# cselab/odil

Measured on AMD Instinct MI355X. Metric: grid-point-updates/s, Poisson 512^3 multigrid, higher is better.
Workload: dtype f64; 1 GPU; 3D Poisson 512^3 multigrid (9 levels) Adam epoch, 1xMI355X, public operator API (odil.util.optimize_grad on examples/poisson/poisson.py); cells_per_gpu=134217728, levels=9, optimizer=adam lr=0.005, decomposition=none, rccl_ranks=1, exchanges_per_epoch=0

## Files before the change

include/odil_hip.h:

```cpp
#ifndef ODIL_HIP_H
#define ODIL_HIP_H

#include <stddef.h>
#include <stdint.h>

#ifdef __cplusplus
extern "C" {
#endif

#define ODIL_MAX_NDIM 4
#define ODIL_MAX_LEVELS 32
#define ODIL_E_INVAL (-1)
#define ODIL_E_LAUNCH (-2)
#define ODIL_E_NODEV (-3)

const char* odil_last_error(void);
int odil_version(void);
int odil_device_count(void);
size_t odil_reduce_workspace_bytes(void);

int odil_interp_add_f64(const double* coarse, const double* add, double* fine, const int64_t* cshape, int ndim,
                        const char* loc, double coarse_scale, double add_scale, void* stream);
int odil_interp_add_f32(const float* coarse, const float* add, float* fine, const int64_t* cshape, int ndim,
                        const char* loc, float coarse_scale, float add_scale, void* stream);
// ... 84 lines not shown
int odil_poisson_residual_restrict_slab_f64(const double* u, const double* rhs, double* coarse, const int64_t* shape,
                                            int ndim, const double* h2, double scale, int64_t z0, int64_t z1,
                                            double denom, double* partials, double* loss, void* stream);
int odil_poisson_residual_restrict_slab_f32(const float* u, const float* rhs, float* coarse, const int64_t* shape,
                                            int ndim, const float* h2, float scale, int64_t z0, int64_t z1, double denom,
                                            double* partials, float* loss, void* stream);
int odil_poisson_adjoint_transpose_adam_f64(const double* fu, double* g0, double* g1, const int64_t* fshape,
                                            const double* h2, double scale, double* x0, double* m0, double* v0,
                                            double* x1, double* m1, double* v1, double alpha, double one_minus_b1,
                                            double one_minus_b2, double eps, const double* alpha_dev, int cut_lo,
                                            int cut_hi, void* stream);
int odil_poisson_adjoint_transpose_adam_f32(const float* fu, float* g0, float* g1, const int64_t* fshape,
                                            const float* h2, float scale, float* x0, float* m0, float* v0, float* x1,
                                            float* m1, float* v1, float alpha, float one_minus_b1, float one_minus_b2,
                                            float eps, const float* alpha_dev, int cut_lo, int cut_hi, void* stream);
int odil_poisson_jacobi_f64(const double* u, const double* rhs, double* uout, const int64_t* shape, int ndim,
                            const double* h2, double omega, void* stream);
int odil_poisson_jacobi_f32(const float* u, const float* rhs, float* uout, const int64_t* shape, int ndim,
                            const float* h2, float omega, void* stream);

int odil_poisson_jacobi2_f64(const double* u, const double* rhs, double* uout, const int64_t* shape, int ndim,
                             const double* h2, double omega1, double omega2, int zc_hint, void* stream);
int odil_poisson_jacobi2_f32(const float* u, const float* rhs, float* uout, const int64_t* shape, int ndim,
                             const float* h2, float omega1, float omega2, int zc_hint, void* stream);

int odil_poisson_jacobi2_synth_f64(const double* coarse, const double* x, const double* rhs, double* xout,
                                   const int64_t* cshape, const double* h2, double omega1, double omega2, int zc_hint,
                                   void* stream);
int odil_poisson_jacobi2_synth_f32(const float* coarse, const float* x, const float* rhs, float* xout,
                                   const int64_t* cshape, const float* h2, float omega1, float omega2, int zc_hint,
// ... 267 lines not shown
```

odil_amd/_lib.py:

```python

import ctypes
import os
from ctypes import c_char_p, c_double, c_float, c_int, c_int64, c_size_t, c_void_p

import numpy as np
import torch

_HERE = os.path.dirname(os.path.abspath(__file__))
LIB_PATH = os.environ.get("ODIL_HIP_LIB") or os.path.join(_HERE, "libodil_hip.so")

_P = c_void_p
_I64P = ctypes.POINTER(c_int64)

_R = "real"
_SIGNATURES = {
    "interp_add": [_P, _P, _P, _I64P, c_int, c_char_p, _R, _R, _P],
    "interp_adj": [_P, _P, _P, _I64P, c_int, c_char_p, _R, _P],
    "interp_add_ld": [_P, c_int64, _P, _P, _I64P, c_int, c_char_p, _R, _R, _P],
    "interp_adj_ld": [_P, _P, c_int64, _I64P, c_int, c_char_p, _P],
    "interp_adj_cut": [_P, _P, _P, _I64P, c_int, c_char_p, _R, c_int, c_int, _P],
    "interp_adj_cut_adam": [_P, _P, _I64P, c_int, c_char_p, c_int, c_int, _P, _P, _P, _R, _R, _R, _R, _P, _P],
    "restrict": [_P, _P, _I64P, c_int, c_char_p, _P],
    "restrict_adj": [_P, _P, _I64P, c_int, c_char_p, _P],
    "conv_valid": [_P, _P, _P, _I64P, _I64P, _I64P, _I64P, c_int, c_int, _P],
# ... 16 lines not shown
    "poisson_adjoint_adam_volumes": [_P, _P, _P, _P, _P, c_int, c_int64, c_int64, c_int64, c_int64, c_int64, _I64P, c_int,
                                     _P, _R, _R, _R, _R, _P, c_int64, _P],
    "mg_synth_adj_adam_volumes": [_P, _P, _I64P, c_int, c_int, c_int, _P, _P, _P, _R, _R, _R, _P, c_int64, _P],
    "poisson_jacobi": [_P, _P, _P, _I64P, c_int, _P, _R, _P],
    "poisson_jacobi2": [_P, _P, _P, _I64P, c_int, _P, _R, _R, c_int, _P],
    "poisson_jacobi2_synth": [_P, _P, _P, _P, _I64P, _P, _R, _R, c_int, _P],
    "poisson_residual_restrict": [_P, _P, _P, _I64P, c_int, _P, _R, _P, _P, _P],
    "poisson_residual_restrict_slab": [_P, _P, _P, _I64P, c_int, _P, _R, c_int64, c_int64, c_double, _P, _P, _P],
    "poisson_residual_synth": [_P, _P, _P, _P, _I64P, _P, c_int64, c_int64, c_double, _P, _P, c_size_t, _P, _P],
    "poisson_jacobi_synth": [_P, _P, _P, _P, _I64P, _P, _R, _P],
    "poisson_residual_slab": [_P, _P, _P, _I64P, c_int, _P, c_int64, c_int64, c_double, _P, _P, _P],
    "poisson_adjoint": [_P, _P, _I64P, c_int, _P, _R, _P],
    "poisson_adjoint_adam": [_P, _P, _P, _P, _P, _I64P, c_int, _P, _R, _R, _R, _R, _R, _P, _P],
    "poisson_adjoint_transpose_adam": [_P, _P, _P, _I64P, _P, _R, _P, _P, _P, _P, _P, _P, _R, _R, _R, _R, _P, c_int,
                                       c_int, _P],
    "poisson_jac_coeffs": [_P, _I64P, c_int, _P, _P],
    "poisson_jac_match": [_P, _I64P, c_int, _P, _P, _P, _P],
    "adam_step": [_P, _P, _P, _P, c_int64, _R, _R, _R, _R, _P, _P],
    "adam_step_pieces": [_P, _P, _P, _P, c_int64, c_int64, c_int64, c_int64, _R, _R, _R, _R, _P, _P],
    "planes_copy": [_P, _P, _P, c_int, c_int64, c_int, c_int, _P],
    "axpy": [_P, _P, c_int64, _R, _P],
    "scale": [_P, _P, c_int64, _R, _P, _P],
    "addcmul": [_P, _P, _P, c_int64, c_int, _P],
    "dots": [_P, c_int64, c_int, _P, c_int64, _P, _P, _P],
    "dots3": [_P, c_int64, c_int, _P, _P, _P, c_int64, _P, _P, _P],
    "lbfgs_probe": [_P, _P, c_int64, _P, _P, _P],
    "lincomb": [_P, _R, _P, c_int64, c_int, _P, c_int64, _P],
    "stencil_apply": [_P, _I64P, c_int, _P, _P, _I64P, c_int, c_int, _P],
    "stencil_march": [_P, _I64P, c_int, c_int, _P, _P, _I64P, c_int, c_int, c_int, _P],
    "stencil_var_smooth": [_P, _P, _P, _P, _I64P, c_int, _R, c_int, _P],
# ... 16 lines not shown
    "bmg_transfer": [_I64P, _I64P, _P, _P, _P, _P, c_int, _P],
    "bmg_galerkin": [_I64P, _I64P, _P, _P, _P, _P, c_int, c_int64, _P, _P],
}

_SIGNATURES_F64 = {
    "bmg_coarse_dense": [_P, _P, _I64P, c_int64, c_int64, _P, _P],
    "bmg_coarse_chol": [_P, c_int64, c_int64, c_double, _P, _P, _P, _P],
}

EXPORTED = [
    "odil_last_error", "odil_version", "odil_device_count", "odil_reduce_workspace_bytes", "odil_dots_workspace_bytes",
    "odil_dense_block_workspace_bytes", "odil_dense_block_wide_workspace_bytes", "odil_narrow_scale", "odil_widen_axpy",
    "odil_poisson_small_epochs_resident", "odil_poisson_small_epochs_partials", "odil_poisson_batch_partials",
    "odil_mg_batch_levels_ok", "odil_poisson_residual_synth_workspace_bytes",
    "odil_mg_volumes_levels_ok", "odil_interp_adj_kind", "odil_poisson_residual_synth_batch_workspace_bytes",
    "odil_poisson_residual_synth_batch_partials", "odil_stencil_solve_batch_work",
] + [
    "odil_{}_{}".format(name, suffix) for name in _SIGNATURES for suffix in ("f64", "f32")
] + ["odil_{}_f64".format(name) for name in _SIGNATURES_F64]

_lib = None


class OdilHipError(RuntimeError):
    pass


def load():
    global _lib
    if _lib is not None:
        return _lib
# ... 21 lines not shown
    lib.odil_poisson_batch_partials.argtypes = [_I64P, c_int, c_int]
    lib.odil_mg_batch_levels_ok.restype = c_int
    lib.odil_mg_batch_levels_ok.argtypes = [_I64P, c_int, c_int, c_int]
    lib.odil_poisson_residual_synth_workspace_bytes.restype = c_size_t
    lib.odil_poisson_residual_synth_workspace_bytes.argtypes = [_I64P]
    lib.odil_interp_adj_kind.restype = c_int
    lib.odil_interp_adj_kind.argtypes = [_I64P, c_int, c_char_p, c_int]
    lib.odil_mg_volumes_levels_ok.restype = c_int
    lib.odil_mg_volumes_levels_ok.argtypes = [_I64P, c_int, c_int, c_int, c_int]
    lib.odil_poisson_residual_synth_batch_workspace_bytes.restype = c_size_t
    lib.odil_poisson_residual_synth_batch_workspace_bytes.argtypes = [_I64P]
    lib.odil_poisson_residual_synth_batch_partials.restype = c_int64
    lib.odil_poisson_residual_synth_batch_partials.argtypes = [_I64P]
    lib.odil_stencil_solve_batch_work.restype = c_int64
    lib.odil_stencil_solve_batch_work.argtypes = [_I64P, c_int, c_int]
    for name in ("odil_narrow_scale", "odil_widen_axpy"):
        fn = getattr(lib, name)
        fn.restype = c_int
        fn.argtypes = [_P, _P, c_int64, c_double, _P, _P]
    for name, sig in _SIGNATURES.items():
        for suffix, real in (("f64", c_double), ("f32", c_float)):
            fn = getattr(lib, "odil_{}_{}".format(name, suffix))
            fn.restype = c_int
            fn.argtypes = [real if a is _R else a for a in sig]
    for name, sig in _SIGNATURES_F64.items():
        fn = getattr(lib, "odil_{}_f64".format(name))
        fn.restype = c_int
        fn.argtypes = sig
    _lib = lib
    return lib
# ... 71 lines not shown
```

odil_amd/csrc/common.h:

```cpp
#pragma once

#include <hip/hip_runtime.h>
#include <stdint.h>
#include <stdio.h>
#include <string.h>

#include "odil_hip.h"

namespace odil {

constexpr int kNumXcd = 8;
constexpr int kBlock = 256;
constexpr int kMaxPartials = 65536;
constexpr int kDotPartials = 1024;
constexpr int64_t kStreamBytes = (int64_t)128 << 20;
constexpr int kGridCap = 2048;

void set_error(const char* fmt, ...);

inline int check_launch(const char* what) {
  hipError_t err = hipGetLastError();
  if (err != hipSuccess) {
    set_error("%s: %s", what, hipGetErrorString(err));
    return ODIL_E_LAUNCH;
// ... 58 lines not shown
  int64_t per_xcd = (int64_t)s.Z * s.Yc * s.XS;
  int64_t cap = kGridCap / kNumXcd;
  if (per_xcd > cap) per_xcd = cap;
  if (per_xcd < 1) per_xcd = 1;
  return (int)(per_xcd * kNumXcd);
}

struct UnitSched {
  int ZCH, Y, XS;
  int ZC;
  int axis;
  int chunk;
  int per_xcd;
};

inline UnitSched make_unit_sched_chunked(int64_t Z, int64_t Y, int64_t XS, int zc) {
  UnitSched s;
  s.ZC = zc;
  s.ZCH = (int)((Z + zc - 1) / zc);
  s.Y = (int)Y;
  s.XS = (int)XS;
  if (Y >= 4 * kNumXcd) {
    s.axis = 1;
    s.chunk = (int)((Y + kNumXcd - 1) / kNumXcd);
    s.per_xcd = s.ZCH * s.chunk * s.XS;
  } else if (s.ZCH >= kNumXcd) {
    s.axis = 0;
    s.chunk = 0;
    s.per_xcd = (int)(((int64_t)s.ZCH * s.Y * s.XS + kNumXcd - 1) / kNumXcd);
  } else {
    s.axis = -1;
    s.chunk = 0;
    s.per_xcd = s.ZCH * s.Y * s.XS;
  }
  return s;
}

inline UnitSched make_unit_sched(int64_t Z, int64_t Y, int64_t XS, int64_t target_units = 2 * kGridCap) {
  int64_t zc = (Z * Y * XS) / target_units;
  if (zc < 1) zc = 1;
  if (zc > 64) zc = 64;
  if (zc > Z) zc = Z;
  return make_unit_sched_chunked(Z, Y, XS, (int)zc);
}

inline int unit_grid(const UnitSched& s) { return s.axis < 0 ? s.per_xcd : s.per_xcd * kNumXcd; }

#ifdef __HIPCC__
__device__ inline bool unit_decode(const UnitSched& s, int& zc, int& y, int& xs) {
  if (s.axis < 0) {
    const int i = blockIdx.x;
    xs = i % s.XS;
    const int r = i / s.XS;
    y = r % s.Y;
    zc = r / s.Y;
    return true;
  }
  const int k = blockIdx.x % kNumXcd, i = blockIdx.x / kNumXcd;
  xs = i % s.XS;
  const int r = i / s.XS;
  if (s.axis == 1) {
    y = k * s.chunk + r % s.chunk;
    zc = r / s.chunk;
    return y < s.Y;
  }
  const int u = k * s.per_xcd + i;
  xs = u % s.XS;
  const int ru = u / s.XS;
  y = ru % s.Y;
  zc = ru / s.Y;
  return zc < s.ZCH;
}
#endif

#ifdef __HIPCC__
struct RowIter {
  int t, step, count, y0, ny;
};

__device__ inline RowIter sched_begin(const RowSched& s) {
  RowIter it;
  const int k = blockIdx.x % kNumXcd;
  it.t = blockIdx.x / kNumXcd;
  it.step = gridDim.x / kNumXcd;
  it.y0 = k * s.Yc;
  int y1 = it.y0 + s.Yc;
  if (y1 > s.Y) y1 = s.Y;
  it.ny = y1 > it.y0 ? y1 - it.y0 : 0;
// ... 78 lines not shown
```

odil_amd/csrc/mg_march.hip:

```cpp
#include "mg_march.h"
#include "poisson.h"

namespace odil {

template <typename T, int CX>
__device__ inline void acc_plane(T (&s)[2][2 * CX], const T (&v)[3][CX + 2], int wz) {
#pragma unroll
  for (int sy = 0; sy < 2; ++sy)
#pragma unroll
    for (int sx = 0; sx < 2 * CX; ++sx) {
      T t = s[sy][sx];
#pragma unroll
      for (int ry = 0; ry < 2; ++ry)
#pragma unroll
        for (int rx = 0; rx < 2; ++rx) {
          const int w = wz * (sy == ry ? 1 : 3) * ((sx & 1) == rx ? 1 : 3);
          t = t + T(w) * v[sy + ry][(sx >> 1) + (sx & 1) + rx];
        }
      s[sy][sx] = t;
    }
}

template <typename T, int CX>
__device__ inline void zero_plane(T (&s)[2][2 * CX]) {
// ... 846 lines not shown
                                           typename TileVec<T, CX>::type (&pre)[2][kTileLoads], T (&wc)[CX][6],
                                           T (&wr)[CX][6], const AdamArgs<T>& ad, const float* __restrict__ wt) {
  __syncthreads();
#pragma unroll
  for (int i = 0; i < kTileLoads; ++i) {
    tile0[dst[i]] = pre[0][i];
    tile1[dst[i]] = pre[1][i];
  }
  __syncthreads();
  tile_fetch<T, CX>(c.gfine, 2 * (c.z0 - 1 + k + ahead), c.fnz, c.fplane, src, pre);
  tile_reduce_emit<T, CX>(c, tile0, tile1, k, live, wc, wr, ad, wt);
}

template <typename T, int CX>
__global__ __launch_bounds__(kBlock) void k_interp_adj_tile(const T* __restrict__ gfine, T* __restrict__ gcoarse,
                                                            T* __restrict__ gscaled, MarchArgs a, T scale,
                                                            AdamArgs<T> ad) {
  typedef typename TileVec<T, CX>::type P2;
  constexpr int NV = 2 * CX;
  __shared__ P2 tile[2][kTileLds];
  __shared__ float wtab[12 * (CX + 1) * kBlock];
  const int cny = a.cn[1], fny = a.fn[1], fnx = a.fn[2];
  int zc, yt, xt;
  if (!unit_decode(a.usched, zc, yt, xt)) return;
  TileCtx<T> c;
  c.cnz = a.cn[0], c.cnx = a.cn[2], c.fnz = a.fn[0];
  c.cut_lo = a.cut_lo, c.cut_hi = a.cut_hi;
  c.cplane = (int64_t)cny * c.cnx, c.fplane = (int64_t)fny * fnx;
  const int64_t cvol = (int64_t)blockIdx.y * c.cnz * c.cplane, fvol = (int64_t)blockIdx.y * c.fnz * c.fplane;
  gfine += fvol;
  c.gfine = gfine, c.gcoarse = gcoarse + cvol, c.gscaled = gscaled ? gscaled + cvol : nullptr;
  if (ad.x) ad.x += cvol, ad.m += cvol, ad.v += cvol;
  if (ad.alpha_dev) ad.alpha_dev += (int64_t)blockIdx.y * ad.alpha_stride;
  c.scale = scale;
  c.z0 = zc * a.usched.ZC;
  const int z1 = c.z0 + a.usched.ZC < c.cnz ? c.z0 + a.usched.ZC : c.cnz;
  tile_column(c.lx, c.ly);
  c.jy = yt * kTileY + c.ly, c.jx = (xt * kTileX + c.lx) * CX;
  c.owner = c.jy < cny && c.jx < c.cnx;
  c.cny = cny;
  c.sx = c.owner && (c.jx < 2 || c.jx + CX - 1 >= c.cnx - 2);
  c.sy = c.owner && (c.jy < 2 || c.jy >= cny - 2);
  if (c.sx || c.sy) {
    Adj6 ax[CX];
    column_taps<CX>(c.jx, c.cnx, ax);
    tile_tables_store<CX>(wtab, adj6(c.jy, cny), ax);
  }
  int64_t src[kTileLoads];
  int dst[kTileLoads];
#pragma unroll
  for (int k = 0; k < kTileLoads; ++k) {
// ... 50 lines not shown
      const int p = threadIdx.x + i * kBlock;
      if (p < kFuPacks) slot[p] = scale * pre[q][i];
    }
  }
}

template <typename T, bool MUL>
__device__ __forceinline__ T lap_inner(T fb, T fm, T fp, const H2<T>& h, int ax) {
  const T s = (fp + fm) + T(-2) * fb;
  if constexpr (MUL) return s * h.inv[ax];
  return div_h2<T>(s, h, ax);
}

template <typename T, bool MUL, bool G0>
__global__ __launch_bounds__(kBlock) void k_poisson_adjoint_tile(const T* __restrict__ fu, T* __restrict__ g0out_,
                                                                 T* __restrict__ gcoarse, MarchArgs a, H2<T> h,
                                                                 T scale, AdamArgs<T> ad0, T* __restrict__ x1,
                                                                 T* __restrict__ m1, T* __restrict__ v1) {
  T* const g0out = G0 ? g0out_ : nullptr;
  AdamArgs<T> ad1 = ad0;
  ad1.x = x1, ad1.m = m1, ad1.v = v1;
  typedef typename TileVec<T>::type P2;
  __shared__ P2 ring[4 * kFuPacks];
  __shared__ P2 gt[2][kTileR * kTileRS];
  const int cny = a.cn[1], fny = a.fn[1], fnx = a.fn[2];
  int zc, yt, xt;
  if (!unit_decode(a.usched, zc, yt, xt)) return;
  if constexpr (MUL) h.mul_ok[0] = h.mul_ok[1] = h.mul_ok[2] = 1;
  if (ad0.alpha_dev) ad0.alpha = *ad0.alpha_dev;
  ad0.alpha_dev = nullptr;
  ad1.alpha = ad0.alpha, ad1.alpha_dev = nullptr;
  TileCtx<T> c;
  c.gfine = nullptr, c.gcoarse = gcoarse, c.gscaled = nullptr;
  c.cnz = a.cn[0], c.cnx = a.cn[2], c.fnz = a.fn[0];
  c.cut_lo = a.cut_lo, c.cut_hi = a.cut_hi;
  c.cplane = (int64_t)cny * c.cnx, c.fplane = (int64_t)fny * fnx;
  c.scale = T(1);
  c.z0 = zc * a.usched.ZC;
  const int z1 = c.z0 + a.usched.ZC < c.cnz ? c.z0 + a.usched.ZC : c.cnz;
  tile_column(c.lx, c.ly);
  c.jy = yt * kTileY + c.ly, c.jx = xt * kTileX + c.lx;
  c.owner = c.jy < cny && c.jx < c.cnx;
  c.cny = cny;
  c.sx = c.owner && (c.jx < 2 || c.jx >= c.cnx - 2);
  c.sy = c.owner && (c.jy < 2 || c.jy >= cny - 2);
  const int fy0 = 2 * yt * kTileY, fx0 = 2 * xt * kTileX;
  const bool tile_inner = fy0 >= 4 && fy0 + 2 * kTileY + 4 <= fny && fx0 >= 4 && fx0 + 2 * kTileX + 4 <= fnx;
  int64_t src[kFuLoads];
#pragma unroll
  for (int i = 0; i < kFuLoads; ++i) {
    int p = threadIdx.x + i * kBlock;
    p = p < kFuPacks ? p : kFuPacks - 1;
    const int r = p / kFuC, cc = p - r * kFuC;
    int fy = fy0 - 3 + r, fx = fx0 - 4 + 2 * cc;
// ... 542 lines not shown
template <typename T>
static bool adj_rows_launch(const T* gfine, T* gcoarse, T* gscaled, const MarchArgs& m, T scale, hipStream_t stream,
                            const AdamArgs<T>& ad) {
  if constexpr (sizeof(T) != 4) {
    return false;
  } else {
    RowsArgs r;
    if (!adj_rows_plan<T>(m, aligned_to(gfine, 16), aligned_to(gcoarse, 8), r)) return false;
    hipLaunchKernelGGL(k_interp_adj_rows, dim3((unsigned)(r.per_xcd * kNumXcd)), dim3(kBlock), 0, stream, gfine, gcoarse,
                       gscaled, r, scale, ad);
    return true;
  }
}

template <typename T>
static void launch_adj_tile(dim3 grid, bool wide, hipStream_t stream, const T* gfine, T* gcoarse, T* gscaled,
                            const MarchArgs& m, T scale, const AdamArgs<T>& ad) {
  if constexpr (sizeof(T) == 4) {
    if (wide) {
      hipLaunchKernelGGL((k_interp_adj_tile<T, 2>), grid, dim3(kBlock), 0, stream, gfine, gcoarse, gscaled, m, scale, ad);
      return;
    }
  }
  hipLaunchKernelGGL((k_interp_adj_tile<T, 1>), grid, dim3(kBlock), 0, stream, gfine, gcoarse, gscaled, m, scale, ad);
}

static bool adj_tile_enabled() {
  const char* e = getenv("ODIL_ADJ_TILE");
  return !e || atoi(e) != 0;
}

static bool adj_small_level(const InterpArgs& a) { return a.cn[0] * a.cn[1] * a.cn[2] * a.cn[3] <= ((int64_t)1 << 22); }

static bool adj_tile_serves(const MarchArgs& m, const InterpArgs& a, int cx) {
  return cx == 1 && m.cn[1] >= 2 * kTileY && m.cn[2] >= 2 * kTileX && adj_tile_enabled() && !a.coarse_ld;
}

template <typename T>
int interp_adj_kind(const InterpArgs& a) {
// ... 17 lines not shown
  const dim3 grid(unit_grid(m.usched), m.lead_cn);
  const bool tile_ok = adj_tile_serves(m, a, CX);
  const bool tile_wide = sizeof(T) == 4 && m.cn[2] % 2 == 0 && m.cn[2] >= 4 * kTileX && aligned_to(gfine, 16);
  const int tile_cols = kTileX * (tile_wide ? 2 : 1);
  if (m.lead_fn != 1) {
    if (m.lead_loc == kNode)
      hipLaunchKernelGGL((k_interp_adj_march_lead<T, CX, 3>), grid, dim3(kBlock), 0, stream, gfine, gcoarse, gscaled,
                         m, scale, ad);
    else if (adj_rows_launch<T>(gfine, gcoarse, gscaled, m, scale, stream, ad)) {
    } else if (tile_ok) {
      const int64_t ytiles = (m.cn[1] + kTileY - 1) / kTileY, xtiles = (m.cn[2] + tile_cols - 1) / tile_cols;
      m.tx = kTileX;
      m.ty = kTileY;
      const int64_t per_volume = kGridCap / m.lead_cn > 2 * ytiles * xtiles ? kGridCap / m.lead_cn : 2 * ytiles * xtiles;
      m.usched = make_unit_sched(m.cn[0], ytiles, xtiles, per_volume);
      launch_adj_tile<T>(dim3(unit_grid(m.usched), m.lead_cn), tile_wide, stream, gfine, gcoarse, gscaled, m, scale, ad);
    } else
      hipLaunchKernelGGL((k_interp_adj_march_lead<T, CX, 1>), grid, dim3(kBlock), 0, stream, gfine, gcoarse, gscaled,
                         m, scale, ad);
  } else if (a.loc[1] == kNode)
    hipLaunchKernelGGL((k_interp_adj_march_n<T, CX>), grid, dim3(kBlock), 0, stream, gfine, gcoarse, gscaled, m, scale,
                       ad);
  else if (adj_rows_launch<T>(gfine, gcoarse, gscaled, m, scale, stream, ad)) {
  } else if (tile_ok) {
    const int64_t ytiles = (m.cn[1] + kTileY - 1) / kTileY, xtiles = (m.cn[2] + tile_cols - 1) / tile_cols;
    m.tx = kTileX;
    m.ty = kTileY;
    m.usched = make_unit_sched(m.cn[0], ytiles, xtiles, small_level ? ODIL_ADJ_UNITS_SMALL : ODIL_TILE_UNITS);
    launch_adj_tile<T>(dim3(unit_grid(m.usched)), tile_wide, stream, gfine, gcoarse, gscaled, m, scale, ad);
  } else
    hipLaunchKernelGGL((k_interp_adj_march<T, CX>), grid, dim3(kBlock), 0, stream, gfine, gcoarse, gscaled, m, scale,
                       ad);
  const int e = check_launch("k_interp_adj_march");
  return e ? e : 1;
}

template <typename T>
int poisson_adjoint_transpose(const T* fu, T* g0, T* g1, const int64_t* fshape, const T* h2, T scale,
                              const AdamArgs<T>& ad0, const AdamArgs<T>& ad1, int cut_lo, int cut_hi,
                              hipStream_t stream) {
  if (!fu || !g1 || !fshape || !h2) {
    set_error("poisson_adjoint_transpose: null pointer (fu, g1, shape, h2)");
    return ODIL_E_INVAL;
  }
  MarchArgs m;
  for (int i = 0; i < 3; ++i) {
    if (fshape[i] < 4 || fshape[i] % 2 || fshape[i] >= (1 << 30)) {
      set_error("poisson_adjoint_transpose: extent %lld on axis %d must be even, >= 4", (long long)fshape[i], i);
      return ODIL_E_INVAL;
    }
    m.fn[i] = (int)fshape[i];
    m.cn[i] = (int)(fshape[i] / 2);
  }
  const void* ptrs[] = {fu, g0, g1, ad0.x, ad0.m, ad0.v};
  for (const void* q : ptrs)
    if (q && !aligned_to(q, 2 * sizeof(T))) {
      set_error("poisson_adjoint_transpose: arrays must be aligned to %d bytes", (int)(2 * sizeof(T)));
      return ODIL_E_INVAL;
    }
  m.tx = kTileX, m.ty = kTileY;
  m.cut_lo = cut_lo, m.cut_hi = cut_hi;
  m.nt = 0;
  m.lead_loc = 0, m.lead_cn = 1, m.lead_fn = 1;
  const int64_t ytiles = (m.cn[1] + kTileY - 1) / kTileY, xtiles = (m.cn[2] + kTileX - 1) / kTileX;
  if ((int64_t)m.cn[0] * ytiles * xtiles >= ((int64_t)1 << 31)) {
    set_error("poisson_adjoint_transpose: grid too large for one launch");
    return ODIL_E_INVAL;
  }
  m.usched = make_unit_sched(m.cn[0], ytiles, xtiles, 2 * kGridCap);
  T h[3] = {h2[0], h2[1], h2[2]};
  const H2<T> hh = make_h2<T>(h);
  const bool mul = hh.mul_ok[0] && hh.mul_ok[1] && hh.mul_ok[2];
  const dim3 grid(unit_grid(m.usched));
#define ODIL_LAUNCH_ADJ_TILE(MUL, G0)                                                                             \
  hipLaunchKernelGGL((k_poisson_adjoint_tile<T, MUL, G0>), grid, dim3(kBlock), 0, stream, fu, g0, g1, m, hh, scale, \
                     ad0, ad1.x, ad1.m, ad1.v)
  if (mul && !g0) ODIL_LAUNCH_ADJ_TILE(true, false);
  else if (mul) ODIL_LAUNCH_ADJ_TILE(true, true);
  else if (!g0) ODIL_LAUNCH_ADJ_TILE(false, false);
  else ODIL_LAUNCH_ADJ_TILE(false, true);
#undef ODIL_LAUNCH_ADJ_TILE
  return check_launch("k_poisson_adjoint_tile");
}

template int poisson_adjoint_transpose<double>(const double*, double*, double*, const int64_t*, const double*, double,
                                               const AdamArgs<double>&, const AdamArgs<double>&, int, int, hipStream_t);
template int poisson_adjoint_transpose<float>(const float*, float*, float*, const int64_t*, const float*, float,
                                              const AdamArgs<float>&, const AdamArgs<float>&, int, int, hipStream_t);

template <typename T>
int interp_add_march(const T* coarse, const T* add, T* fine, const InterpArgs& a, T cscale, T ascale,
                     hipStream_t stream) {
  const int cx = march_cx<T>(a, fine, add);
  if constexpr (sizeof(T) == 4) {
    if (cx == 2) return add_launch<T, 2>(coarse, add, fine, a, cscale, ascale, stream);
  }
  return cx ? add_launch<T, 1>(coarse, add, fine, a, cscale, ascale, stream) : 0;
}

template <typename T>
int interp_adj_march(const T* gfine, T* gcoarse, T* gscaled, const InterpArgs& a, T scale, hipStream_t stream,
                     const AdamArgs<T>& ad) {
  return march_cx<T>(a, gfine, nullptr) ? adj_launch<T, 1>(gfine, gcoarse, gscaled, a, scale, stream, ad) : 0;
}

template int interp_add_march<double>(const double*, const double*, double*, const InterpArgs&, double, double,
                                      hipStream_t);
template int interp_add_march<float>(const float*, const float*, float*, const InterpArgs&, float, float, hipStream_t);
template int interp_adj_march<double>(const double*, double*, double*, const InterpArgs&, double, hipStream_t,
                                      const AdamArgs<double>&);
template int interp_adj_march<float>(const float*, float*, float*, const InterpArgs&, float, hipStream_t,
                                     const AdamArgs<float>&);

}

using namespace odil;

extern "C" {
int odil_poisson_adjoint_transpose_adam_f64(const double* fu, double* g0, double* g1, const int64_t* fshape,
                                            const double* h2, double scale, double* x0, double* m0, double* v0,
                                            double* x1, double* m1, double* v1, double alpha, double one_minus_b1,
                                            double one_minus_b2, double eps, const double* alpha_dev, int cut_lo,
                                            int cut_hi, void* stream) {
  const AdamArgs<double> a0{x0, m0, v0, alpha, one_minus_b1, one_minus_b2, eps, alpha_dev};
  const AdamArgs<double> a1{x1, m1, v1, alpha, one_minus_b1, one_minus_b2, eps, alpha_dev};
  return poisson_adjoint_transpose<double>(fu, g0, g1, fshape, h2, scale, a0, a1, cut_lo, cut_hi, (hipStream_t)stream);
}
int odil_poisson_adjoint_transpose_adam_f32(const float* fu, float* g0, float* g1, const int64_t* fshape,
                                            const float* h2, float scale, float* x0, float* m0, float* v0, float* x1,
                                            float* m1, float* v1, float alpha, float one_minus_b1, float one_minus_b2,
                                            float eps, const float* alpha_dev, int cut_lo, int cut_hi, void* stream) {
  const AdamArgs<float> a0{x0, m0, v0, alpha, one_minus_b1, one_minus_b2, eps, alpha_dev};
  const AdamArgs<float> a1{x1, m1, v1, alpha, one_minus_b1, one_minus_b2, eps, alpha_dev};
  return poisson_adjoint_transpose<float>(fu, g0, g1, fshape, h2, scale, a0, a1, cut_lo, cut_hi, (hipStream_t)stream);
}
}
```

odil_amd/ops.py:

```python

import math
from ctypes import c_double, c_int, c_int64, c_size_t, c_void_p

import torch

from . import _lib
from ._lib import call, host_reals, i64, ptr, ptr_array, stream_ptr

_workspace = {}


def reduce_workspace(device, nquant=1):
    key = (str(device), nquant)
    ws = _workspace.get(key)
    if ws is None:
        ws = torch.empty(_lib.reduce_workspace_elems() * nquant, dtype=torch.float64, device=device)
        _workspace[key] = ws
    return ws


_column_sums = {}


def residual_synth_workspace(device, cshape):
# ... 677 lines not shown
    assert x.shape == fu.shape and m.numel() == v.numel() == fu.numel()
    h2a, h2p = host_reals(h2, fu.dtype)
    a, adev = _step_size(alpha, fu.dtype)
    call(
        "poisson_adjoint_adam", fu.dtype, ptr(fu), ptr(out), ptr(x), ptr(m), ptr(v), i64(fu.shape), c_int(fu.dim()),
        h2p, float(scale), a, float(one_minus_b1), float(one_minus_b2), float(eps), adev, stream_ptr(),
    )
    return out


def adjoint_transpose_supported(shape):
    return len(shape) == 3 and all(n % 2 == 0 for n in shape) and shape[0] >= 8 and shape[1] >= 32 and shape[2] >= 128


def poisson_adjoint_transpose(fu, h2, scale, g1, g0=None, adam0=None, adam1=None, alpha=0.0, one_minus_b1=0.0,
                              one_minus_b2=0.0, eps=0.0, cut=(False, False)):
    assert fu.dim() == 3 and tuple(g1.shape) == tuple(n // 2 for n in fu.shape) and fu.is_contiguous()
    h2a, h2p = host_reals(h2, fu.dtype)
    a, adev = _step_size(alpha, fu.dtype)
    a0 = adam0 if adam0 is not None else (None, None, None)
    a1 = adam1 if adam1 is not None else (None, None, None)
    for t in list(a0) + list(a1):
        assert t is None or (t.is_contiguous() and t.dtype == fu.dtype)
    call(
        "poisson_adjoint_transpose_adam", fu.dtype, ptr(fu), ptr(g0), ptr(g1), i64(fu.shape), h2p, float(scale),
        ptr(a0[0]), ptr(a0[1]), ptr(a0[2]), ptr(a1[0]), ptr(a1[1]), ptr(a1[2]), a, float(one_minus_b1),
        float(one_minus_b2), float(eps), adev, c_int(1 if cut[0] else 0), c_int(1 if cut[1] else 0), stream_ptr(),
    )
    return g1


def poisson_jac_match(arrays, shape, h2):
    from ._lib import ptr_array

    ndim = len(shape)
    assert len(arrays) == 2 * ndim + 1 and all(a.numel() == math.prod(shape) for a in arrays)
    arrays = [a.reshape(-1) if a.is_contiguous() else a.reshape(-1).contiguous() for a in arrays]
    dtype = arrays[0].dtype
    h2a, h2p = host_reals(h2, dtype)
    out = torch.empty((2 * ndim + 1, 2), dtype=dtype, device=arrays[0].device)
    call("poisson_jac_match", dtype, ptr_array(arrays), i64(shape), c_int(ndim), h2p, ptr(reduce_workspace(out.device)), ptr(out),
         stream_ptr())
    return out

# ... 275 lines not shown
```

Baseline: 54.02 billion grid-point-updates/s.

## Split adjoint tile z-chunks into long bulk and short tail tiers

```diff
diff --git a/include/odil_hip.h b/include/odil_hip.h
--- a/include/odil_hip.h
+++ b/include/odil_hip.h
@@ -122,6 +122,19 @@
                                             const float* h2, float scale, float* x0, float* m0, float* v0, float* x1,
                                             float* m1, float* v1, float alpha, float one_minus_b1, float one_minus_b2,
                                             float eps, const float* alpha_dev, int cut_lo, int cut_hi, void* stream);
+int odil_poisson_adjoint_transpose_adam_plan_f64(const double* fu, double* g0, double* g1, const int64_t* fshape,
+                                                 const double* h2, double scale, double* x0, double* m0, double* v0,
+                                                 double* x1, double* m1, double* v1, double alpha, double one_minus_b1,
+                                                 double one_minus_b2, double eps, const double* alpha_dev, int cut_lo,
+                                                 int cut_hi, int L, int Zs, int S, void* stream);
+int odil_poisson_adjoint_transpose_adam_plan_f32(const float* fu, float* g0, float* g1, const int64_t* fshape,
+                                                 const float* h2, float scale, float* x0, float* m0, float* v0, float* x1,
+                                                 float* m1, float* v1, float alpha, float one_minus_b1,
+                                                 float one_minus_b2, float eps, const float* alpha_dev, int cut_lo,
+                                                 int cut_hi, int L, int Zs, int S, void* stream);
+int odil_tile_sched_rule(const int64_t* fshape, int kind, int* plan);
+int64_t odil_tile_sched_units(int64_t Z, int64_t Y, int64_t XS, int L, int64_t Zs, int S, int32_t* units,
+                              int64_t capacity);
 int odil_poisson_jacobi_f64(const double* u, const double* rhs, double* uout, const int64_t* shape, int ndim,
                             const double* h2, double omega, void* stream);
 int odil_poisson_jacobi_f32(const float* u, const float* rhs, float* uout, const int64_t* shape, int ndim,
diff --git a/odil_amd/_lib.py b/odil_amd/_lib.py
--- a/odil_amd/_lib.py
+++ b/odil_amd/_lib.py
@@ -54,6 +54,8 @@
     "poisson_adjoint_adam": [_P, _P, _P, _P, _P, _I64P, c_int, _P, _R, _R, _R, _R, _R, _P, _P],
     "poisson_adjoint_transpose_adam": [_P, _P, _P, _I64P, _P, _R, _P, _P, _P, _P, _P, _P, _R, _R, _R, _R, _P, c_int,
                                        c_int, _P],
+    "poisson_adjoint_transpose_adam_plan": [_P, _P, _P, _I64P, _P, _R, _P, _P, _P, _P, _P, _P, _R, _R, _R, _R, _P, c_int,
+                                            c_int, c_int, c_int, c_int, _P],
     "poisson_jac_coeffs": [_P, _I64P, c_int, _P, _P],
     "poisson_jac_match": [_P, _I64P, c_int, _P, _P, _P, _P],
     "adam_step": [_P, _P, _P, _P, c_int64, _R, _R, _R, _R, _P, _P],
@@ -100,7 +102,8 @@
     "odil_poisson_small_epochs_resident", "odil_poisson_small_epochs_partials", "odil_poisson_batch_partials",
     "odil_mg_batch_levels_ok", "odil_poisson_residual_synth_workspace_bytes",
     "odil_mg_volumes_levels_ok", "odil_interp_adj_kind", "odil_poisson_residual_synth_batch_workspace_bytes",
-    "odil_poisson_residual_synth_batch_partials", "odil_stencil_solve_batch_work",
+    "odil_poisson_residual_synth_batch_partials", "odil_stencil_solve_batch_work", "odil_tile_sched_rule",
+    "odil_tile_sched_units",
 ] + [
     "odil_{}_{}".format(name, suffix) for name in _SIGNATURES for suffix in ("f64", "f32")
 ] + ["odil_{}_f64".format(name) for name in _SIGNATURES_F64]
@@ -152,6 +155,10 @@
     lib.odil_poisson_residual_synth_batch_partials.argtypes = [_I64P]
     lib.odil_stencil_solve_batch_work.restype = c_int64
     lib.odil_stencil_solve_batch_work.argtypes = [_I64P, c_int, c_int]
+    lib.odil_tile_sched_rule.restype = c_int
+    lib.odil_tile_sched_rule.argtypes = [_I64P, c_int, ctypes.POINTER(c_int)]
+    lib.odil_tile_sched_units.restype = c_int64
+    lib.odil_tile_sched_units.argtypes = [c_int64, c_int64, c_int64, c_int, c_int64, c_int, _P, c_int64]
     for name in ("odil_narrow_scale", "odil_widen_axpy"):
         fn = getattr(lib, name)
         fn.restype = c_int
diff --git a/odil_amd/csrc/common.h b/odil_amd/csrc/common.h
--- a/odil_amd/csrc/common.h
+++ b/odil_amd/csrc/common.h
@@ -96,10 +96,10 @@
   int per_xcd;
 };
 
-inline UnitSched make_unit_sched_chunked(int64_t Z, int64_t Y, int64_t XS, int zc) {
+inline UnitSched make_unit_sched_of_chunks(int64_t nchunks, int64_t Y, int64_t XS, int zc) {
   UnitSched s;
   s.ZC = zc;
-  s.ZCH = (int)((Z + zc - 1) / zc);
+  s.ZCH = (int)nchunks;
   s.Y = (int)Y;
   s.XS = (int)XS;
   if (Y >= 4 * kNumXcd) {
@@ -118,6 +118,10 @@
   return s;
 }
 
+inline UnitSched make_unit_sched_chunked(int64_t Z, int64_t Y, int64_t XS, int zc) {
+  return make_unit_sched_of_chunks((Z + zc - 1) / zc, Y, XS, zc);
+}
+
 inline UnitSched make_unit_sched(int64_t Z, int64_t Y, int64_t XS, int64_t target_units = 2 * kGridCap) {
   int64_t zc = (Z * Y * XS) / target_units;
   if (zc < 1) zc = 1;
@@ -129,16 +133,21 @@
 inline int unit_grid(const UnitSched& s) { return s.axis < 0 ? s.per_xcd : s.per_xcd * kNumXcd; }
 
 #ifdef __HIPCC__
-__device__ inline bool unit_decode(const UnitSched& s, int& zc, int& y, int& xs) {
+#define ODIL_HD __host__ __device__
+#else
+#define ODIL_HD
+#endif
+
+ODIL_HD inline bool unit_decode_at(const UnitSched& s, int b, int& zc, int& y, int& xs) {
   if (s.axis < 0) {
-    const int i = blockIdx.x;
+    const int i = b;
     xs = i % s.XS;
     const int r = i / s.XS;
     y = r % s.Y;
     zc = r / s.Y;
     return true;
   }
-  const int k = blockIdx.x % kNumXcd, i = blockIdx.x / kNumXcd;
+  const int k = b % kNumXcd, i = b / kNumXcd;
   xs = i % s.XS;
   const int r = i / s.XS;
   if (s.axis == 1) {
@@ -153,7 +162,43 @@
   zc = ru / s.Y;
   return zc < s.ZCH;
 }
-#endif
+
+#ifdef __HIPCC__
+__device__ inline bool unit_decode(const UnitSched& s, int& zc, int& y, int& xs) {
+  return unit_decode_at(s, (int)blockIdx.x, zc, y, xs);
+}
+#endif
+
+struct TierSched {
+  UnitSched u;
+  int Z, Zs;
+  int S;
+  int NL;
+};
+
+inline bool tier_plan_ok(int64_t Z, int L, int64_t Zs, int S) { return S >= 1 && S <= L && Zs >= 0 && Zs <= Z; }
+
+inline TierSched make_tier_sched(int64_t Z, int64_t Y, int64_t XS, int L, int64_t Zs, int S) {
+  if (L > Z) L = (int)Z;
+  if (S > L) S = L;
+  if (Zs == 0) L = S;
+  if (L == S || Zs >= Z) Zs = Z, S = L;
+  TierSched t;
+  t.Z = (int)Z, t.Zs = (int)Zs, t.S = S;
+  t.NL = (int)((Zs + L - 1) / L);
+  t.u = make_unit_sched_of_chunks(t.NL + (Z - Zs + S - 1) / S, Y, XS, L);
+  return t;
+}
+
+ODIL_HD inline bool tier_decode_at(const TierSched& t, int b, int& z0, int& z1, int& y, int& xs) {
+  int zc;
+  if (!unit_decode_at(t.u, b, zc, y, xs)) return false;
+  const bool lng = zc < t.NL;
+  const int len = lng ? t.u.ZC : t.S, end = lng ? t.Zs : t.Z;
+  z0 = lng ? zc * len : t.Zs + (zc - t.NL) * len;
+  z1 = z0 + len < end ? z0 + len : end;
+  return true;
+}
 
 #ifdef __HIPCC__
 struct RowIter {
diff --git a/odil_amd/csrc/mg_march.hip b/odil_amd/csrc/mg_march.hip
--- a/odil_amd/csrc/mg_march.hip
+++ b/odil_amd/csrc/mg_march.hip
@@ -884,15 +884,15 @@
 
 template <typename T, int CX>
 __global__ __launch_bounds__(kBlock) void k_interp_adj_tile(const T* __restrict__ gfine, T* __restrict__ gcoarse,
-                                                            T* __restrict__ gscaled, MarchArgs a, T scale,
-                                                            AdamArgs<T> ad) {
+                                                            T* __restrict__ gscaled, MarchArgs a, TierSched ts,
+                                                            T scale, AdamArgs<T> ad) {
   typedef typename TileVec<T, CX>::type P2;
   constexpr int NV = 2 * CX;
   __shared__ P2 tile[2][kTileLds];
   __shared__ float wtab[12 * (CX + 1) * kBlock];
   const int cny = a.cn[1], fny = a.fn[1], fnx = a.fn[2];
-  int zc, yt, xt;
-  if (!unit_decode(a.usched, zc, yt, xt)) return;
+  int z0, z1, yt, xt;
+  if (!tier_decode_at(ts, (int)blockIdx.x, z0, z1, yt, xt)) return;
   TileCtx<T> c;
   c.cnz = a.cn[0], c.cnx = a.cn[2], c.fnz = a.fn[0];
   c.cut_lo = a.cut_lo, c.cut_hi = a.cut_hi;
@@ -903,8 +903,7 @@
   if (ad.x) ad.x += cvol, ad.m += cvol, ad.v += cvol;
   if (ad.alpha_dev) ad.alpha_dev += (int64_t)blockIdx.y * ad.alpha_stride;
   c.scale = scale;
-  c.z0 = zc * a.usched.ZC;
-  const int z1 = c.z0 + a.usched.ZC < c.cnz ? c.z0 + a.usched.ZC : c.cnz;
+  c.z0 = z0;
   tile_column(c.lx, c.ly);
   c.jy = yt * kTileY + c.ly, c.jx = (xt * kTileX + c.lx) * CX;
   c.owner = c.jy < cny && c.jx < c.cnx;
@@ -985,8 +984,8 @@
 
 template <typename T, bool MUL, bool G0>
 __global__ __launch_bounds__(kBlock) void k_poisson_adjoint_tile(const T* __restrict__ fu, T* __restrict__ g0out_,
-                                                                 T* __restrict__ gcoarse, MarchArgs a, H2<T> h,
-                                                                 T scale, AdamArgs<T> ad0, T* __restrict__ x1,
+                                                                 T* __restrict__ gcoarse, MarchArgs a, TierSched ts,
+                                                                 H2<T> h, T scale, AdamArgs<T> ad0, T* __restrict__ x1,
                                                                  T* __restrict__ m1, T* __restrict__ v1) {
   T* const g0out = G0 ? g0out_ : nullptr;
   AdamArgs<T> ad1 = ad0;
@@ -995,8 +994,8 @@
   __shared__ P2 ring[4 * kFuPacks];
   __shared__ P2 gt[2][kTileR * kTileRS];
   const int cny = a.cn[1], fny = a.fn[1], fnx = a.fn[2];
-  int zc, yt, xt;
-  if (!unit_decode(a.usched, zc, yt, xt)) return;
+  int z0, z1, yt, xt;
+  if (!tier_decode_at(ts, (int)blockIdx.x, z0, z1, yt, xt)) return;
   if constexpr (MUL) h.mul_ok[0] = h.mul_ok[1] = h.mul_ok[2] = 1;
   if (ad0.alpha_dev) ad0.alpha = *ad0.alpha_dev;
   ad0.alpha_dev = nullptr;
@@ -1007,8 +1006,7 @@
   c.cut_lo = a.cut_lo, c.cut_hi = a.cut_hi;
   c.cplane = (int64_t)cny * c.cnx, c.fplane = (int64_t)fny * fnx;
   c.scale = T(1);
-  c.z0 = zc * a.usched.ZC;
-  const int z1 = c.z0 + a.usched.ZC < c.cnz ? c.z0 + a.usched.ZC : c.cnz;
+  c.z0 = z0;
   tile_column(c.lx, c.ly);
   c.jy = yt * kTileY + c.ly, c.jx = xt * kTileX + c.lx;
   c.owner = c.jy < cny && c.jx < c.cnx;
@@ -1581,15 +1579,41 @@
 }
 
 template <typename T>
-static void launch_adj_tile(dim3 grid, bool wide, hipStream_t stream, const T* gfine, T* gcoarse, T* gscaled,
+static void launch_adj_tile(const TierSched& ts, bool wide, hipStream_t stream, const T* gfine, T* gcoarse, T* gscaled,
                             const MarchArgs& m, T scale, const AdamArgs<T>& ad) {
+  const dim3 grid(unit_grid(ts.u), m.lead_cn);
   if constexpr (sizeof(T) == 4) {
     if (wide) {
-      hipLaunchKernelGGL((k_interp_adj_tile<T, 2>), grid, dim3(kBlock), 0, stream, gfine, gcoarse, gscaled, m, scale, ad);
+      hipLaunchKernelGGL((k_interp_adj_tile<T, 2>), grid, dim3(kBlock), 0, stream, gfine, gcoarse, gscaled, m, ts, scale,
+                         ad);
       return;
     }
   }
-  hipLaunchKernelGGL((k_interp_adj_tile<T, 1>), grid, dim3(kBlock), 0, stream, gfine, gcoarse, gscaled, m, scale, ad);
+  hipLaunchKernelGGL((k_interp_adj_tile<T, 1>), grid, dim3(kBlock), 0, stream, gfine, gcoarse, gscaled, m, ts, scale, ad);
+}
+
+constexpr int kTileSlots = 512;
+constexpr int kTierShort = 4, kTierTailRounds = 2, kTierBulkRounds = 4;
+
+static void tile_plan_rule(int64_t Z, int64_t ytiles, int64_t xtiles, int64_t target_units, int& L, int64_t& Zs, int& S) {
+  const UnitSched one = make_unit_sched(Z, ytiles, xtiles, target_units);
+  L = S = one.ZC, Zs = Z;
+  const int64_t tiles = ytiles * xtiles;
+  if (one.axis != 1 || one.ZC <= kTierShort || (int64_t)one.ZCH * tiles < 2 * kTileSlots) return;
+  const int64_t short_chunks = kTierTailRounds * kTileSlots / tiles > 1 ? kTierTailRounds * kTileSlots / tiles : 1;
+  const int64_t tail = kTierShort * short_chunks;
+  if (tail + one.ZC > Z) return;
+  const int64_t round_planes = (int64_t)kTileSlots * kTierBulkRounds;
+  int64_t len = (Z * tiles + round_planes - 1) / round_planes;
+  len = len < one.ZC ? one.ZC : (len > 64 ? 64 : len);
+  L = (int)len, Zs = Z - tail, S = kTierShort;
+}
+
+static TierSched tile_plan(int64_t Z, int64_t ytiles, int64_t xtiles, int64_t target_units) {
+  int L, S;
+  int64_t Zs;
+  tile_plan_rule(Z, ytiles, xtiles, target_units, L, Zs, S);
+  return make_tier_sched(Z, ytiles, xtiles, L, Zs, S);
 }
 
 static bool adj_tile_enabled() {
@@ -1637,7 +1661,8 @@
       m.ty = kTileY;
       const int64_t per_volume = kGridCap / m.lead_cn > 2 * ytiles * xtiles ? kGridCap / m.lead_cn : 2 * ytiles * xtiles;
       m.usched = make_unit_sched(m.cn[0], ytiles, xtiles, per_volume);
-      launch_adj_tile<T>(dim3(unit_grid(m.usched), m.lead_cn), tile_wide, stream, gfine, gcoarse, gscaled, m, scale, ad);
+      launch_adj_tile<T>(make_tier_sched(m.cn[0], ytiles, xtiles, m.usched.ZC, m.cn[0], m.usched.ZC), tile_wide, stream,
+                         gfine, gcoarse, gscaled, m, scale, ad);
     } else
       hipLaunchKernelGGL((k_interp_adj_march_lead<T, CX, 1>), grid, dim3(kBlock), 0, stream, gfine, gcoarse, gscaled,
                          m, scale, ad);
@@ -1649,8 +1674,9 @@
     const int64_t ytiles = (m.cn[1] + kTileY - 1) / kTileY, xtiles = (m.cn[2] + tile_cols - 1) / tile_cols;
     m.tx = kTileX;
     m.ty = kTileY;
-    m.usched = make_unit_sched(m.cn[0], ytiles, xtiles, small_level ? ODIL_ADJ_UNITS_SMALL : ODIL_TILE_UNITS);
-    launch_adj_tile<T>(dim3(unit_grid(m.usched)), tile_wide, stream, gfine, gcoarse, gscaled, m, scale, ad);
+    const TierSched ts = tile_plan(m.cn[0], ytiles, xtiles, small_level ? ODIL_ADJ_UNITS_SMALL : ODIL_TILE_UNITS);
+    m.usched = ts.u;
+    launch_adj_tile<T>(ts, tile_wide, stream, gfine, gcoarse, gscaled, m, scale, ad);
   } else
     hipLaunchKernelGGL((k_interp_adj_march<T, CX>), grid, dim3(kBlock), 0, stream, gfine, gcoarse, gscaled, m, scale,
                        ad);
@@ -1661,7 +1687,7 @@
 template <typename T>
 int poisson_adjoint_transpose(const T* fu, T* g0, T* g1, const int64_t* fshape, const T* h2, T scale,
                               const AdamArgs<T>& ad0, const AdamArgs<T>& ad1, int cut_lo, int cut_hi,
-                              hipStream_t stream) {
+                              hipStream_t stream, const int* plan) {
   if (!fu || !g1 || !fshape || !h2) {
     set_error("poisson_adjoint_transpose: null pointer (fu, g1, shape, h2)");
     return ODIL_E_INVAL;
@@ -1690,13 +1716,24 @@
     set_error("poisson_adjoint_transpose: grid too large for one launch");
     return ODIL_E_INVAL;
   }
-  m.usched = make_unit_sched(m.cn[0], ytiles, xtiles, 2 * kGridCap);
+  TierSched ts;
+  if (plan) {
+    if (!tier_plan_ok(m.cn[0], plan[0], plan[1], plan[2]) || plan[0] > 64) {
+      set_error("poisson_adjoint_transpose: plan (L %d, Zs %d, S %d) needs 1 <= S <= L <= 64, 0 <= Zs <= %d", plan[0],
+                plan[1], plan[2], m.cn[0]);
+      return ODIL_E_INVAL;
+    }
+    ts = make_tier_sched(m.cn[0], ytiles, xtiles, plan[0], plan[1], plan[2]);
+  } else {
+    ts = tile_plan(m.cn[0], ytiles, xtiles, 2 * kGridCap);
+  }
+  m.usched = ts.u;
   T h[3] = {h2[0], h2[1], h2[2]};
   const H2<T> hh = make_h2<T>(h);
   const bool mul = hh.mul_ok[0] && hh.mul_ok[1] && hh.mul_ok[2];
-  const dim3 grid(unit_grid(m.usched));
-#define ODIL_LAUNCH_ADJ_TILE(MUL, G0)                                                                             \
-  hipLaunchKernelGGL((k_poisson_adjoint_tile<T, MUL, G0>), grid, dim3(kBlock), 0, stream, fu, g0, g1, m, hh, scale, \
+  const dim3 grid(unit_grid(ts.u));
+#define ODIL_LAUNCH_ADJ_TILE(MUL, G0)                                                                                 \
+  hipLaunchKernelGGL((k_poisson_adjoint_tile<T, MUL, G0>), grid, dim3(kBlock), 0, stream, fu, g0, g1, m, ts, hh, scale, \
                      ad0, ad1.x, ad1.m, ad1.v)
   if (mul && !g0) ODIL_LAUNCH_ADJ_TILE(true, false);
   else if (mul) ODIL_LAUNCH_ADJ_TILE(true, true);
@@ -1707,9 +1744,23 @@
 }
 
 template int poisson_adjoint_transpose<double>(const double*, double*, double*, const int64_t*, const double*, double,
-                                               const AdamArgs<double>&, const AdamArgs<double>&, int, int, hipStream_t);
+                                               const AdamArgs<double>&, const AdamArgs<double>&, int, int, hipStream_t,
+                                               const int*);
 template int poisson_adjoint_transpose<float>(const float*, float*, float*, const int64_t*, const float*, float,
-                                              const AdamArgs<float>&, const AdamArgs<float>&, int, int, hipStream_t);
+                                              const AdamArgs<float>&, const AdamArgs<float>&, int, int, hipStream_t,
+                                              const int*);
+
+static int tile_sched_rule(const int64_t* fshape, int kind, int* plan) {
+  const int64_t Z = fshape[0] / 2, cny = fshape[1] / 2, cnx = fshape[2] / 2;
+  const int64_t ytiles = (cny + kTileY - 1) / kTileY, xtiles = (cnx + kTileX - 1) / kTileX;
+  const bool small_level = Z * cny * cnx <= ((int64_t)1 << 22);
+  int L, S;
+  int64_t Zs;
+  tile_plan_rule(Z, ytiles, xtiles, kind == 0 ? 2 * kGridCap : (small_level ? ODIL_ADJ_UNITS_SMALL : ODIL_TILE_UNITS), L, Zs,
+                 S);
+  plan[0] = L, plan[1] = (int)Zs, plan[2] = S;
+  return 0;
+}
 
 template <typename T>
 int interp_add_march(const T* coarse, const T* add, T* fine, const InterpArgs& a, T cscale, T ascale,
@@ -1740,21 +1791,58 @@
 using namespace odil;
 
 extern "C" {
+int odil_poisson_adjoint_transpose_adam_plan_f64(const double* fu, double* g0, double* g1, const int64_t* fshape,
+                                                 const double* h2, double scale, double* x0, double* m0, double* v0,
+                                                 double* x1, double* m1, double* v1, double alpha, double one_minus_b1,
+                                                 double one_minus_b2, double eps, const double* alpha_dev, int cut_lo,
+                                                 int cut_hi, int L, int Zs, int S, void* stream) {
+  const AdamArgs<double> a0{x0, m0, v0, alpha, one_minus_b1, one_minus_b2, eps, alpha_dev};
+  const AdamArgs<double> a1{x1, m1, v1, alpha, one_minus_b1, one_minus_b2, eps, alpha_dev};
+  const int plan[3] = {L, Zs, S};
+  return poisson_adjoint_transpose<double>(fu, g0, g1, fshape, h2, scale, a0, a1, cut_lo, cut_hi, (hipStream_t)stream,
+                                           L > 0 ? plan : nullptr);
+}
+int odil_poisson_adjoint_transpose_adam_plan_f32(const float* fu, float* g0, float* g1, const int64_t* fshape,
+                                                 const float* h2, float scale, float* x0, float* m0, float* v0, float* x1,
+                                                 float* m1, float* v1, float alpha, float one_minus_b1,
+                                                 float one_minus_b2, float eps, const float* alpha_dev, int cut_lo,
+                                                 int cut_hi, int L, int Zs, int S, void* stream) {
+  const AdamArgs<float> a0{x0, m0, v0, alpha, one_minus_b1, one_minus_b2, eps, alpha_dev};
+  const AdamArgs<float> a1{x1, m1, v1, alpha, one_minus_b1, one_minus_b2, eps, alpha_dev};
+  const int plan[3] = {L, Zs, S};
+  return poisson_adjoint_transpose<float>(fu, g0, g1, fshape, h2, scale, a0, a1, cut_lo, cut_hi, (hipStream_t)stream,
+                                          L > 0 ? plan : nullptr);
+}
 int odil_poisson_adjoint_transpose_adam_f64(const double* fu, double* g0, double* g1, const int64_t* fshape,
                                             const double* h2, double scale, double* x0, double* m0, double* v0,
                                             double* x1, double* m1, double* v1, double alpha, double one_minus_b1,
                                             double one_minus_b2, double eps, const double* alpha_dev, int cut_lo,
                                             int cut_hi, void* stream) {
-  const AdamArgs<double> a0{x0, m0, v0, alpha, one_minus_b1, one_minus_b2, eps, alpha_dev};
-  const AdamArgs<double> a1{x1, m1, v1, alpha, one_minus_b1, one_minus_b2, eps, alpha_dev};
-  return poisson_adjoint_transpose<double>(fu, g0, g1, fshape, h2, scale, a0, a1, cut_lo, cut_hi, (hipStream_t)stream);
+  return odil_poisson_adjoint_transpose_adam_plan_f64(fu, g0, g1, fshape, h2, scale, x0, m0, v0, x1, m1, v1, alpha,
+                                                      one_minus_b1, one_minus_b2, eps, alpha_dev, cut_lo, cut_hi, 0, 0, 0,
+                                                      stream);
 }
 int odil_poisson_adjoint_transpose_adam_f32(const float* fu, float* g0, float* g1, const int64_t* fshape,
                                             const float* h2, float scale, float* x0, float* m0, float* v0, float* x1,
                                             float* m1, float* v1, float alpha, float one_minus_b1, float one_minus_b2,
                                             float eps, const float* alpha_dev, int cut_lo, int cut_hi, void* stream) {
-  const AdamArgs<float> a0{x0, m0, v0, alpha, one_minus_b1, one_minus_b2, eps, alpha_dev};
-  const AdamArgs<float> a1{x1, m1, v1, alpha, one_minus_b1, one_minus_b2, eps, alpha_dev};
-  return poisson_adjoint_transpose<float>(fu, g0, g1, fshape, h2, scale, a0, a1, cut_lo, cut_hi, (hipStream_t)stream);
-}
-}
+  return odil_poisson_adjoint_transpose_adam_plan_f32(fu, g0, g1, fshape, h2, scale, x0, m0, v0, x1, m1, v1, alpha,
+                                                      one_minus_b1, one_minus_b2, eps, alpha_dev, cut_lo, cut_hi, 0, 0, 0,
+                                                      stream);
+}
+int odil_tile_sched_rule(const int64_t* fshape, int kind, int* plan) {
+  if (!fshape || !plan || fshape[0] < 4 || fshape[1] < 4 || fshape[2] < 4 || kind < 0 || kind > 1) return ODIL_E_INVAL;
+  return tile_sched_rule(fshape, kind, plan);
+}
+int64_t odil_tile_sched_units(int64_t Z, int64_t Y, int64_t XS, int L, int64_t Zs, int S, int32_t* units, int64_t capacity) {
+  if (Z < 1 || Y < 1 || XS < 1 || !tier_plan_ok(Z, L, Zs, S)) return -1;
+  const TierSched ts = make_tier_sched(Z, Y, XS, L, Zs, S);
+  const int64_t grid = unit_grid(ts.u);
+  for (int64_t b = 0; units && b < grid && b < capacity; ++b) {
+    int z0 = -1, z1 = -1, y = -1, xs = -1;
+    if (!tier_decode_at(ts, (int)b, z0, z1, y, xs)) z0 = z1 = y = xs = -1;
+    units[4 * b] = z0, units[4 * b + 1] = z1, units[4 * b + 2] = y, units[4 * b + 3] = xs;
+  }
+  return grid;
+}
+}
diff --git a/odil_amd/ops.py b/odil_amd/ops.py
--- a/odil_amd/ops.py
+++ b/odil_amd/ops.py
@@ -1,6 +1,6 @@
 
 import math
-from ctypes import c_double, c_int, c_int64, c_size_t, c_void_p
+from ctypes import c_double, c_int, c_int32, c_int64, c_size_t, c_void_p
 
 import torch
 
@@ -715,7 +715,7 @@
 
 
 def poisson_adjoint_transpose(fu, h2, scale, g1, g0=None, adam0=None, adam1=None, alpha=0.0, one_minus_b1=0.0,
-                              one_minus_b2=0.0, eps=0.0, cut=(False, False)):
+                              one_minus_b2=0.0, eps=0.0, cut=(False, False), plan=None):
     assert fu.dim() == 3 and tuple(g1.shape) == tuple(n // 2 for n in fu.shape) and fu.is_contiguous()
     h2a, h2p = host_reals(h2, fu.dtype)
     a, adev = _step_size(alpha, fu.dtype)
@@ -723,12 +723,41 @@
     a1 = adam1 if adam1 is not None else (None, None, None)
     for t in list(a0) + list(a1):
         assert t is None or (t.is_contiguous() and t.dtype == fu.dtype)
+    if plan is not None:
+        L, Zs, S = (int(p) for p in plan)
+        if not 1 <= S <= L <= 64 or not 0 <= Zs <= g1.shape[0]:
+            raise ValueError("plan (L, Zs, S) = {} needs 1 <= S <= L <= 64 and 0 <= Zs <= {}".format(plan, g1.shape[0]))
+        call(
+            "poisson_adjoint_transpose_adam_plan", fu.dtype, ptr(fu), ptr(g0), ptr(g1), i64(fu.shape), h2p, float(scale),
+            ptr(a0[0]), ptr(a0[1]), ptr(a0[2]), ptr(a1[0]), ptr(a1[1]), ptr(a1[2]), a, float(one_minus_b1),
+            float(one_minus_b2), float(eps), adev, c_int(1 if cut[0] else 0), c_int(1 if cut[1] else 0), c_int(L),
+            c_int(Zs), c_int(S), stream_ptr(),
+        )
+        return g1
     call(
         "poisson_adjoint_transpose_adam", fu.dtype, ptr(fu), ptr(g0), ptr(g1), i64(fu.shape), h2p, float(scale),
         ptr(a0[0]), ptr(a0[1]), ptr(a0[2]), ptr(a1[0]), ptr(a1[1]), ptr(a1[2]), a, float(one_minus_b1),
         float(one_minus_b2), float(eps), adev, c_int(1 if cut[0] else 0), c_int(1 if cut[1] else 0), stream_ptr(),
     )
     return g1
+
+
+def adjoint_transpose_plan(shape, transpose_only=False):
+    out = (c_int * 3)()
+    if _lib.load().odil_tile_sched_rule(i64(shape), 1 if transpose_only else 0, out) != 0:
+        raise ValueError("adjoint_transpose_plan: shape {}".format(tuple(shape)))
+    return tuple(out)
+
+
+def tile_sched_units(Z, Y, XS, L, Zs, S):
+    lib = _lib.load()
+    grid = lib.odil_tile_sched_units(Z, Y, XS, L, Zs, S, None, 0)
+    if grid < 0:
+        raise ValueError("tile_sched_units: ({}, {}, {}) is not a plan for {} planes".format(L, Zs, S, Z))
+    buf = (c_int32 * (4 * grid))()
+    lib.odil_tile_sched_units(Z, Y, XS, L, Zs, S, buf, grid)
+    flat = list(buf)
+    return [None if flat[4 * b] < 0 else tuple(flat[4 * b:4 * b + 4]) for b in range(grid)]
 
 
 def poisson_jac_match(arrays, shape, h2):
```

Result: faster. 55.23 billion grid-point-updates/s, median of 6 (+2.2%).
